# ocramz/rp-tree

Measured on AMD Instinct MI355X. Metric: forest-build vectors/s (1000000 x 128 dense f64, 32 trees; projection mode mfma = RPT_PROJ_MFMA, the API default RPT_PROJ_AUTO on f64 data is the exact-order kernel timed in `other_projection_mode`); kNN queries/s and recall@10 in `knn` / `recall_at_10`, higher is better.
Workload: dtype f64; 1 GPU; C2: 1000000 x 128 f64 two-Gaussian mixture, 32-tree forest, minLeaf 128, maxDepth 13, pnz 0.4746, k=10, 10000 queries; trees sharded 32/GPU, X replicated; projection_mode=mfma

## Files before the change

### rp-tree_amd/csrc/api.hip

```cpp
#include <cctype>
#include <cmath>
#include <cstdlib>
#include <cstring>
#include <limits>
#include <map>
#include <mutex>
#include <new>

#include "common.h"

namespace rpt {

static thread_local std::string g_err;
void set_error(const std::string& msg) { g_err = msg; }
int32_t fail(int32_t code, const std::string& msg) {
  g_err = msg;
  return code;
}

namespace {
struct Block {
  void* p;
  size_t bytes;
};
// ... 108 lines not shown

int32_t upload_async(rpt_ctx* ctx, void* dst_dev, const void* src_host, size_t bytes) {
  if (bytes == 0) return RPT_OK;
  void* stage = pin_alloc(ctx, bytes);
  if (!stage) {
    RPT_HIP(hipMemcpyAsync(dst_dev, src_host, bytes, hipMemcpyHostToDevice, ctx->stream));
    RPT_HIP(stream_sync(ctx->stream));
    return RPT_OK;
  }
  std::memcpy(stage, src_host, bytes);
  RPT_HIP(hipMemcpyAsync(dst_dev, stage, bytes, hipMemcpyHostToDevice, ctx->stream));
  return RPT_OK;
}

hipError_t ctx_sync(rpt_ctx* ctx) {
  const hipError_t e = stream_sync(ctx->stream);
  ctx->pin_off = 0;
  return e;
}

void dev_trim() {
  int dev = 0;
  (void)hipGetDevice(&dev);
  (void)hipDeviceSynchronize();
  std::lock_guard<std::mutex> lk(g_pool_mu);
  for (size_t i = 0; i < g_pool_pending.size();) {
    if (g_pool_pending[i].dev == dev) {
      (void)hipFree(g_pool_pending[i].p);
      g_pool_pending[i] = g_pool_pending.back();
      g_pool_pending.pop_back();
    } else {
      ++i;
    }
  }
  auto it = g_pool_free.find(dev);
  if (it != g_pool_free.end()) {
    for (Block& b : it->second) (void)hipFree(b.p);
    it->second.clear();
  }
}

void enumerate_topology(int64_t N, int32_t L, int32_t min_leaf, std::vector<Node>& out) {
  struct Item { int32_t level; int64_t heap, off, n; };
  std::vector<Item> stack;
  stack.push_back({0, 0, 0, N});
  while (!stack.empty()) {
    Item it = stack.back();
    stack.pop_back();
    bool leaf = is_leaf(it.level, it.n, L, min_leaf);
    out.push_back({it.level, it.heap, it.off, it.n, leaf});
    if (!leaf) {
      int64_t nh = it.n / 2;
      stack.push_back({it.level + 1, 2 * it.heap + 2, it.off + nh, it.n - nh});
      stack.push_back({it.level + 1, 2 * it.heap + 1, it.off, nh});
    }
  }
}

}

using namespace rpt;

static void prof_resolve(rpt_ctx* ctx);

namespace {
struct OptDesc {
  const char* name;
  int64_t rpt_options::*field;
};
const OptDesc kOptions[] = {
    {"no_stream", &rpt_options::no_stream},
    {"stream_maxnodes", &rpt_options::stream_maxnodes},
    {"stream_minper", &rpt_options::stream_minper},
    {"no_wmid", &rpt_options::no_wmid},
    {"no_midselect", &rpt_options::no_midselect},
    {"stream_big_node", &rpt_options::stream_big_node},
    {"no_wsub", &rpt_options::no_wsub},
    {"no_wsort", &rpt_options::no_wsort},
    {"no_wpack", &rpt_options::no_wpack},
    {"no_csub", &rpt_options::no_csub},
    {"no_codes", &rpt_options::no_codes},
    {"no_pcodes", &rpt_options::no_pcodes},
    {"proj_narrow", &rpt_options::proj_narrow},
    {"proj_bf16_f32", &rpt_options::proj_bf16_f32},
    {"proj_bf16_terms", &rpt_options::proj_bf16_terms},
    {"proj_bf16_codes", &rpt_options::proj_bf16_codes},
    {"proj_csr_nodense", &rpt_options::proj_csr_nodense},
    {"knn_wave", &rpt_options::knn_wave},
    {"knn_kp", &rpt_options::knn_kp},
    {"knn_no_pre32", &rpt_options::knn_no_pre32},
    {"knn_no_pre16", &rpt_options::knn_no_pre16},
    {"knn_kp16", &rpt_options::knn_kp16},
    {"knn_no_pre8", &rpt_options::knn_no_pre8},
    {"knn_kp8", &rpt_options::knn_kp8},
    {"knn_metric_exact", &rpt_options::knn_metric_exact},
    {"knn_csr_pre32", &rpt_options::knn_csr_pre32},
    {"knn_general", &rpt_options::knn_general},
    {"graph_general", &rpt_options::graph_general},
    {"graph_refine_general", &rpt_options::graph_refine_general},
    {"graph_search_nofilter", &rpt_options::graph_search_nofilter},
    {"knn_shard_old", &rpt_options::knn_shard_old},
    {"brute_csr_tile", &rpt_options::brute_csr_tile},
    {"comm_force_exchange", &rpt_options::comm_force_exchange},
    {"comm_inject_failure", &rpt_options::comm_inject_failure},
    {"comm_timeout_ms", &rpt_options::comm_timeout_ms},
    {"comm_stall_test", &rpt_options::comm_stall_test},
    {"tune0", &rpt_options::tune0},
    {"tune1", &rpt_options::tune1},
    {"tune2", &rpt_options::tune2},
    {"tune3", &rpt_options::tune3},
    {"debug_host", &rpt_options::debug_host},
    {"debug_stamps", &rpt_options::debug_stamps},
};
const OptDesc* find_option(const char* name) {
  if (!name) return nullptr;
  for (const OptDesc& o : kOptions)
    if (std::strcmp(o.name, name) == 0) return &o;
  return nullptr;
}
void options_from_env(rpt_options& opt) {
  for (const OptDesc& o : kOptions) {
    std::string env = "RPT_";
    for (const char* c = o.name; *c; ++c) env += (char)std::toupper((unsigned char)*c);
    if (const char* v = getenv(env.c_str())) {
      char* end = nullptr;
      const long long x = std::strtoll(v, &end, 10);
      opt.*(o.field) = (end && end != v) ? (int64_t)x : 1;
    }
  }
}

template <class F>
int32_t guarded(F&& body) noexcept {
  try {
    return body();
  } catch (const std::bad_alloc&) {
    try {
      return fail(RPT_E_NOMEM, "out of host memory");
    } catch (...) {
      return RPT_E_NOMEM;
    }
  } catch (const std::exception& e) {
    try {
      return fail(RPT_E_INTERNAL, std::string("internal error: ") + e.what());
    } catch (...) {
      return RPT_E_INTERNAL;
    }
  } catch (...) {
    return RPT_E_INTERNAL;
  }
}
}

extern "C" {

int32_t rpt_abi_version(void) { return RPT_ABI_VERSION; }
const char* rpt_last_error(void) { return g_err.c_str(); }

int32_t rpt_device_count(int32_t* count) {
  return guarded([&]() -> int32_t {
    RPT_ARG(count, "count is NULL");
    int c = 0;
    hipError_t e = hipGetDeviceCount(&c);
    if (e != hipSuccess) {
      *count = 0;
      return fail(RPT_E_HIP, std::string("hipGetDeviceCount: ") + hipGetErrorString(e));
// ... 1322 lines not shown
```

### rp-tree_amd/csrc/common.h

```cpp
#pragma once

#include <hip/hip_runtime.h>
#include <stdint.h>

#include <atomic>
#include <mutex>
#include <string>
#include <vector>

#include "../../include/rptree_hip.h"

namespace rpt {

void set_error(const std::string& msg);
int32_t fail(int32_t code, const std::string& msg);

#define RPT_HIP(expr)                                                                     \
  do {                                                                                    \
    hipError_t e__ = (expr);                                                              \
    if (e__ != hipSuccess)                                                                \
      return ::rpt::fail(RPT_E_HIP, std::string(#expr) + ": " + hipGetErrorString(e__));  \
  } while (0)

#define RPT_TRY(expr)             \
// ... 18 lines not shown
  return level >= L || n <= (int64_t)min_leaf;
}
void enumerate_topology(int64_t N, int32_t L, int32_t min_leaf, std::vector<Node>& out);

struct Seg {
  int64_t off;
  int32_t n;
  int32_t heap;
};

inline size_t dtype_size(int32_t dt) { return dt == RPT_F64 ? 8 : dt == RPT_F32 ? 4 : 2; }
inline int32_t proj_dtype(int32_t dt) { return dt == RPT_F64 ? RPT_F64 : RPT_F32; }

hipError_t dev_alloc(void** p, size_t bytes);
void dev_free(void* p);
void dev_trim();
void dev_set_stream(hipStream_t s);
hipError_t stream_sync(hipStream_t s);

struct DeviceOnce {
  std::mutex mu;
  std::atomic<unsigned long long> done{0};
  template <class F>
  int32_t run(int dev, F&& f) {
    const unsigned long long bit = 1ULL << (dev & 63);
    if (done.load(std::memory_order_acquire) & bit) return 0;
    std::lock_guard<std::mutex> lk(mu);
    if (done.load(std::memory_order_relaxed) & bit) return 0;
    const int32_t s = f();
    if (s == 0) done.fetch_or(bit, std::memory_order_release);
    return s;
  }
};

template <class T>
struct DevBuf {
  T* p = nullptr;
  size_t count = 0;
  ~DevBuf() { release(); }
  DevBuf() = default;
  DevBuf(const DevBuf&) = delete;
  DevBuf& operator=(const DevBuf&) = delete;
  void release() {
    if (p) dev_free(p);
    p = nullptr;
    count = 0;
  }
  int32_t alloc(size_t n) {
    release();
    if (n == 0) n = 1;
    hipError_t e = dev_alloc((void**)&p, n * sizeof(T));
    if (e != hipSuccess)
      return fail(RPT_E_NOMEM, std::string("hipMalloc failed: ") + hipGetErrorString(e));
    count = n;
    return RPT_OK;
  }
  int32_t ensure(size_t n) { return (n <= count && p) ? RPT_OK : alloc(n); }
};

}

enum { RPT_PROF_PROJECT = 0, RPT_PROF_SPLIT = 1, RPT_PROF_KNN_PLAN = 2, RPT_PROF_KNN_TOPK = 3,
       RPT_PROF_PROJECT_WIDE = 4, RPT_PROF_CLASSES = 5 };

struct rpt_prof_span {
  hipEvent_t a, b;
  int which;
};

struct rpt_options {
  int64_t no_stream = 0;
  int64_t stream_maxnodes = 0;
  int64_t stream_minper = 32768;
  int64_t no_wmid = 0;
  int64_t no_midselect = 0;
  int64_t stream_big_node = (int64_t)1 << 21;
  int64_t no_wsub = 0;
  int64_t no_wsort = 0;
  int64_t no_wpack = 0;
  int64_t no_csub = 0;
  int64_t no_codes = 0;
  int64_t no_pcodes = 0;
  int64_t proj_narrow = 0;
  int64_t proj_bf16_f32 = 0;
  int64_t proj_bf16_codes = 0;
  int64_t proj_bf16_terms = 0;
  int64_t proj_csr_nodense = 0;
  int64_t knn_wave = -1;
  int64_t knn_kp = 0;
  int64_t knn_no_pre32 = 0;
  int64_t knn_no_pre16 = 0;
  int64_t knn_kp16 = 0;
  int64_t knn_no_pre8 = 0;
  int64_t knn_kp8 = 0;
  int64_t knn_metric_exact = 0;
  int64_t knn_csr_pre32 = 0;
  int64_t knn_general = 0;
  int64_t graph_general = 0;
  int64_t graph_refine_general = 0;
  int64_t graph_search_nofilter = 0;
  int64_t brute_csr_tile = 0;
  int64_t knn_shard_old = 0;
  int64_t comm_force_exchange = 0;
  int64_t comm_inject_failure = 0;
  int64_t comm_timeout_ms = 0;
  int64_t comm_stall_test = 0;
  int64_t tune0 = 0, tune1 = 0, tune2 = 0, tune3 = 0;
  int64_t debug_host = 0;
  int64_t debug_stamps = 0;
};

struct rpt_ctx {
  rpt_options opt;
  int32_t device = 0;
  hipStream_t stream = nullptr;
  char* pin = nullptr;
  size_t pin_cap = 0, pin_off = 0;
  int64_t last_uncertified = 0;
  unsigned long long* metric_unc_dev = nullptr;
  bool metric_unc_pending = false;
  int64_t last_candidates = 0;
  int64_t last_retries = 0;
  int64_t last_graph_pairs = 0;
  void* refine_state_dev = nullptr;
  void* search_state_dev = nullptr;
  void* prepare_state_dev = nullptr;
  int32_t last_tier = 0;
  int64_t last_csub_redo = 0, last_csub_bad = 0;
  int32_t n_cu = 256;
  bool prof = false;
  std::vector<rpt_prof_span> spans;
  std::vector<hipEvent_t> prof_events;
  double prof_ms[RPT_PROF_CLASSES] = {0, 0, 0, 0, 0};
  int64_t prof_n[RPT_PROF_CLASSES] = {0, 0, 0, 0, 0};
};

namespace rpt {
struct ProfScope {
  rpt_ctx* ctx;
  rpt_prof_span sp;
  bool on;
  ProfScope(rpt_ctx* c, int which) : ctx(c), on(c->prof) {
    if (!on) return;
    sp.which = which;
    auto take = [&](hipEvent_t& e) {
      if (!ctx->prof_events.empty()) {
        e = ctx->prof_events.back();
        ctx->prof_events.pop_back();
        return true;
      }
      return hipEventCreate(&e) == hipSuccess;
    };
    if (!take(sp.a)) {
      on = false;
      return;
    }
    if (!take(sp.b)) {
      ctx->prof_events.push_back(sp.a);
      on = false;
      return;
    }
    (void)hipEventRecord(sp.a, ctx->stream);
  }
  ~ProfScope() {
    if (!on) return;
    (void)hipEventRecord(sp.b, ctx->stream);
// ... 120 lines not shown
```

### rp-tree_amd/csrc/project.hip

```cpp
#include <hip/hip_bf16.h>

#include <cstdlib>
#include <vector>

#include "common.h"
#include "codes.h"

namespace rpt {
namespace {

typedef double double4_t __attribute__((ext_vector_type(4)));
typedef float float4_t __attribute__((ext_vector_type(4)));

constexpr int kWave = 64;

template <class T>
struct Vec16;
template <>
struct Vec16<double> { typedef double type __attribute__((ext_vector_type(2))); };
template <>
struct Vec16<float> { typedef float type __attribute__((ext_vector_type(4))); };

template <class T>
__global__ void transpose_R(const double* __restrict__ R, int C, int d, int CB,
                            T* __restrict__ Rt) {
  int64_t total = (int64_t)((C + CB - 1) / CB) * d * CB;
  for (int64_t i = blockIdx.x * (int64_t)blockDim.x + threadIdx.x; i < total;
       i += (int64_t)gridDim.x * blockDim.x) {
    int c = (int)(i % CB);
    int k = (int)((i / CB) % d);
    int blk = (int)(i / ((int64_t)CB * d));
    int col = blk * CB + c;
    Rt[i] = col < C ? (T)R[(int64_t)col * d + k] : (T)0;
  }
}

__device__ inline double mul_rn(double a, double b) { return __dmul_rn(a, b); }
__device__ inline double add_rn(double a, double b) { return __dadd_rn(a, b); }
__device__ inline float mul_rn(float a, float b) { return __fmul_rn(a, b); }
__device__ inline float add_rn(float a, float b) { return __fadd_rn(a, b); }
__device__ inline double fma_rn(double a, double b, double c) { return __builtin_fma(a, b, c); }
__device__ inline float fma_rn(float a, float b, float c) { return __builtin_fmaf(a, b, c); }

template <class T, int CB, int KC>
__global__ __launch_bounds__(256) void proj_exact(const T* __restrict__ X, int64_t n, int d,
                                                  const T* __restrict__ Rt ,
                                                  T* __restrict__ P, int64_t ldp, int ncol) {
  constexpr int LDW = KC + 1;
  __shared__ T tile[4][kWave * LDW];
  const int lane = threadIdx.x & 63;
  const int wave = threadIdx.x >> 6;
  const int64_t row0 = ((int64_t)blockIdx.x * 4 + wave) * kWave;
  T* my = tile[wave];

  T acc[CB];
#pragma unroll
  for (int c = 0; c < CB; ++c) acc[c] = (T)0;

  const int nchunk = (d + KC - 1) / KC;
  for (int ch = nchunk - 1; ch >= 0; --ch) {
    const int k0 = ch * KC;
    const int klen = min(KC, d - k0);
    __syncthreads();
    for (int e = lane; e < kWave * KC; e += kWave) {
      int r = e / KC, k = e % KC;
      int64_t row = row0 + r;
      T v = (T)0;
      if (k < klen && row < n) v = X[row * d + k0 + k];
      my[r * LDW + k] = v;
    }
    __syncthreads();
    const T* rrow = Rt + (int64_t)k0 * CB;
    for (int k = klen - 1; k >= 0; --k) {
      const T x = my[lane * LDW + k];
      const T* rk = rrow + (int64_t)k * CB;
#pragma unroll
      for (int c = 0; c < CB; ++c) acc[c] = add_rn(mul_rn(rk[c], x), acc[c]);
    }
  }
  const int64_t row = row0 + lane;
  if (row < n) {
#pragma unroll
    for (int c = 0; c < CB; ++c)
      if (c < ncol) P[(int64_t)c * ldp + row] = acc[c];
  }
// ... 213 lines not shown
  const int hi = __builtin_amdgcn_mov_dpp((int)(b >> 32), 0xb1, 0xf, 0xf, true);
  return __longlong_as_double(((long long)hi << 32) | (unsigned int)lo);
}
__device__ __forceinline__ float lane_swap1(float x) {
  return __int_as_float(__builtin_amdgcn_mov_dpp(__float_as_int(x), 0xb1, 0xf, 0xf, true));
}

template <class TC, int CBT, bool CODES>
__device__ __forceinline__ void tile_store(const typename Mfma<TC>::acc_t (&acc)[CBT], TC* __restrict__ P,
                                           int64_t ldp, int c0, int ncol, int64_t row0, int64_t n,
                                           int lane, const CodeCtl<TC>* ctl, unsigned int cmask) {
  const int64_t r4 = row0 + 4 * (lane >> 4);
  if constexpr (sizeof(TC) == 8) {
    const bool whole = row0 + 15 < n && (ldp & 1) == 0 && ncol == CBT * 16;
    if (whole) {
      typedef double d2 __attribute__((ext_vector_type(2), aligned(16)));
      const int odd = lane & 1;
#pragma unroll
      for (int h = 0; h < CBT; ++h) {
        const double g0 = odd ? acc[h][0] : acc[h][2], g1 = odd ? acc[h][1] : acc[h][3];
        const double x0 = lane_swap1(g0), x1 = lane_swap1(g1);
        const int col = h * 16 + (lane & 15);
        TC* pe = P + (int64_t)(c0 + (col & ~1)) * ldp + r4 + 2 * odd;
        TC* po = pe + ldp;
        d2 ve, vo;
        if (odd) {
          ve = d2{x0, x1};
          vo = d2{acc[h][2], acc[h][3]};
        } else {
          ve = d2{acc[h][0], acc[h][1]};
          vo = d2{x0, x1};
        }
        *reinterpret_cast<d2*>(pe) = ve;
        *reinterpret_cast<d2*>(po) = vo;
      }
    }
    if (whole) goto codes;
  }
  if (r4 >= n) return;
  {
  const bool vec = r4 + 3 < n && (ldp & 3) == 0;
#pragma unroll
  for (int h = 0; h < CBT; ++h) {
    const int col = h * 16 + (lane & 15);
    if (col < ncol) {
      TC* p = P + (int64_t)(c0 + col) * ldp + r4;
      if (vec) {
        typename Vec4<TC>::type v;
#pragma unroll
        for (int r = 0; r < 4; ++r) v[r] = acc[h][r];
        *reinterpret_cast<typename Vec4<TC>::type*>(p) = v;
      } else {
#pragma unroll
        for (int r = 0; r < 4; ++r)
          if (r4 + r < n) p[r] = acc[h][r];
      }
    }
  }
  }
codes:
  if constexpr (CODES) {
    if (cmask == 0) return;
    const CodeCtl<TC> cc = *ctl;
    const CodeGeo<TC> g{cc.s, cc.b};
    const bool cvec = r4 + 3 < n && (cc.ld & 3) == 0;
#pragma unroll
    for (int h = 0; h < CBT; ++h)
      if ((cmask >> h) & 1u) {
        uint16_t* q = cc.base + (int64_t)(h * 16 + (lane & 15)) * cc.ld + r4;
        if (cvec) {
          code4_t v;
#pragma unroll
          for (int r = 0; r < 4; ++r) v[r] = code_of(acc[h][r], g);
          *reinterpret_cast<code4_t*>(q) = v;
        } else {
#pragma unroll
          for (int r = 0; r < 4; ++r)
            if (r4 + r < n) q[r] = code_of(acc[h][r], g);
        }
      }
  }
}

template <class TIn, class TC, int CBT, int KCH, int WAVES>
__global__ __launch_bounds__(WAVES * 64) void proj_mfma(const TIn* __restrict__ X, int64_t n,
                                                        int d, const double* __restrict__ R,
                                                        int c0, int ncol, TC* __restrict__ P,
                                                        int64_t ldp, int64_t ntiles) {
  constexpr int STEPS = KCH / 4;
  constexpr int LDW = KCH + 16 / (int)sizeof(TC);
  __shared__ __attribute__((aligned(16))) TC tile[WAVES][16 * LDW];
  const int lane = threadIdx.x & 63;
  const int wave = threadIdx.x >> 6;
  const int m = lane & 15, q = lane >> 4;
  TC* my = tile[wave];
  typedef typename Mfma<TC>::acc_t acc_t;

  const int nchunk = (d + KCH - 1) / KCH;
  TC a[CBT][STEPS];
  auto load_a = [&](int k0) {
#pragma unroll
    for (int h = 0; h < CBT; ++h) {
      const int col = h * 16 + m;
#pragma unroll
      for (int s = 0; s < STEPS; ++s) {
        const int k = k0 + 4 * s + q;
        a[h][s] = (col < ncol && k < d) ? (TC)R[(int64_t)(c0 + col) * d + k] : (TC)0;
      }
    }
  };
  if (nchunk == 1) load_a(0);

  const int64_t wave_global = (int64_t)blockIdx.x * WAVES + wave;
  const int64_t wave_stride = (int64_t)gridDim.x * WAVES;
  for (int64_t t = wave_global; t < ntiles; t += wave_stride) {
    const int64_t row0 = t * 16;
    acc_t acc[CBT];
#pragma unroll
    for (int h = 0; h < CBT; ++h) acc[h] = acc_t{0, 0, 0, 0};

    for (int ch = 0; ch < nchunk; ++ch) {
      const int k0 = ch * KCH;
      if (nchunk > 1) load_a(k0);
      constexpr int VEC = 16 / (int)sizeof(TIn);
      const bool vec_ok = (d % VEC) == 0;
      __builtin_amdgcn_wave_barrier();
      if (vec_ok) {
        for (int e = lane; e < 16 * (KCH / VEC); e += 64) {
          const int r = e / (KCH / VEC), kv = (e % (KCH / VEC)) * VEC;
          const int64_t row = row0 + r;
          TC v[VEC];
          if (row < n && k0 + kv < d) {
            struct alignas(16) Raw { TIn v[VEC]; };
            const Raw g = *reinterpret_cast<const Raw*>(X + row * d + k0 + kv);
#pragma unroll
            for (int j = 0; j < VEC; ++j) {
              if constexpr (sizeof(TIn) == sizeof(TC)) v[j] = (TC)g.v[j];
              else v[j] = (TC)to_f32<TIn>(g.v[j]);
            }
          } else {
#pragma unroll
            for (int j = 0; j < VEC; ++j) v[j] = (TC)0;
          }
#pragma unroll
          for (int j = 0; j < VEC; ++j) my[r * LDW + kv + j] = v[j];
        }
      } else {
        for (int e = lane; e < 16 * KCH; e += 64) {
          const int r = e / KCH, k = e % KCH;
          const int64_t row = row0 + r;
          TC v = (TC)0;
          if (row < n && k0 + k < d) {
            if constexpr (sizeof(TIn) == sizeof(TC)) v = (TC)X[row * d + k0 + k];
            else v = (TC)to_f32<TIn>(X[row * d + k0 + k]);
          }
          my[r * LDW + k] = v;
        }
      }
      __builtin_amdgcn_wave_barrier();
      __builtin_amdgcn_fence(__ATOMIC_ACQ_REL, "wavefront");
#pragma unroll
      for (int s = 0; s < STEPS; ++s) {
        const TC b = my[m * LDW + 4 * s + q];
#pragma unroll
        for (int h = 0; h < CBT; ++h) acc[h] = Mfma<TC>::run(a[h][s], b, acc[h]);
      }
    }
    const int64_t row = row0 + m;
    if (row < n) {
#pragma unroll
      for (int h = 0; h < CBT; ++h)
#pragma unroll
        for (int r = 0; r < 4; ++r) {
          const int col = h * 16 + Mfma<TC>::row_of(lane, r);
          if (col < ncol) P[(int64_t)(c0 + col) * ldp + row] = acc[h][r];
        }
    }
  }
}

template <class TC>
__global__ void pad_A_kernel(const double* __restrict__ R, int C, int d, int D, int nblk, int cbt,
                             int col0, int k0, TC* __restrict__ Apad ) {
  const int steps = D / 4;
  const int64_t total = (int64_t)nblk * cbt * steps * 64;
  for (int64_t i = blockIdx.x * (int64_t)blockDim.x + threadIdx.x; i < total;
       i += (int64_t)gridDim.x * blockDim.x) {
    const int lane = (int)(i & 63);
    const int s = (int)((i >> 6) % steps);
    const int h = (int)((i / (64 * (int64_t)steps)) % cbt);
    const int blk = (int)(i / (64 * (int64_t)steps * cbt));
    const int col = col0 + blk * 16 * cbt + h * 16 + (lane & 15);
    const int k = k0 + 4 * s + (lane >> 4);
    Apad[i] = (col < C && k < d) ? (TC)R[(int64_t)col * d + k] : (TC)0;
  }
}

template <class TIn, class TC, int D, int CBT, bool CODES = false>
__device__ __forceinline__ void proj_fast_body(const TIn* __restrict__ X, int64_t n,
                                               const TC* __restrict__ Apad, int c0,
                                               int ncol, TC* __restrict__ P,
                                               int64_t ldp, int64_t ntiles,
                                               int64_t ldx ,
                                               int accumulate ,
                                               int kvalid ,
                                               uint16_t* __restrict__ Cd ,
                                               int64_t ldc,
                                               const unsigned long long* __restrict__ cmm,
                                               int cL, int cLc ) {
  constexpr int STEPS = D / 4;
  constexpr int PIECE = 16 / (int)sizeof(TIn);
  constexpr int PIECES_PER_ROW = D / PIECE;
  __shared__ CodeCtl<TC> cctl;
  unsigned int cmask = 0;
  if constexpr (CODES) {
    if (threadIdx.x == 0) {
      const CodeGeo<TC> g = code_geo<TC>(cmm[0], cmm[1]);
      cctl = CodeCtl<TC>{Cd + (int64_t)c0 * ldc, ldc, g.s, g.b};
    }
    cmask = code_lane_mask<CBT>(threadIdx.x & 63, c0, ncol, cL, cLc);
    __syncthreads();
  }
  constexpr int NP = 16 * PIECES_PER_ROW / 64;
  constexpr int LDW = D + 16 / (int)sizeof(TC);
  static_assert((16 * PIECES_PER_ROW) % 64 == 0, "tile must be a multiple of 64 pieces");
  __shared__ __attribute__((aligned(16))) TC tile[4][16 * LDW];
  const int lane = threadIdx.x & 63;
  const int wave = threadIdx.x >> 6;
  const int m = lane & 15, q = lane >> 4;
  TC* my = tile[wave];
  typedef typename Mfma<TC>::acc_t acc_t;
  struct alignas(16) Raw { TIn v[PIECE]; };

  TC a[CBT][STEPS];
#pragma unroll
  for (int h = 0; h < CBT; ++h)
#pragma unroll
    for (int s = 0; s < STEPS; ++s) a[h][s] = Apad[(h * STEPS + s) * 64 + lane];

  const int64_t wave_global = (int64_t)blockIdx.x * 4 + wave;
  const int64_t wave_stride = (int64_t)gridDim.x * 4;
  const int64_t last_row = n - 1;

  Raw stage[NP];
  auto issue = [&](int64_t t) {
    const int64_t row0 = t * 16;
#pragma unroll
    for (int i = 0; i < NP; ++i) {
      const int p = i * 64 + lane;
      int64_t row = row0 + p / PIECES_PER_ROW;
      row = row < last_row ? row : last_row;
      if ((p % PIECES_PER_ROW) * PIECE < kvalid)
        stage[i] = *reinterpret_cast<const Raw*>(X + row * ldx + (p % PIECES_PER_ROW) * PIECE);
      else
        stage[i] = Raw{};
    }
  };
  auto commit = [&]() {
#pragma unroll
    for (int i = 0; i < NP; ++i) {
      const int p = i * 64 + lane;
      TC* dst = my + (p / PIECES_PER_ROW) * LDW + (p % PIECES_PER_ROW) * PIECE;
#pragma unroll
      for (int j = 0; j < PIECE; ++j) {
        if constexpr (sizeof(TIn) == sizeof(TC)) dst[j] = (TC)stage[i].v[j];
        else dst[j] = (TC)to_f32<TIn>(stage[i].v[j]);
      }
    }
  };

  int64_t t = wave_global;
  if (t < ntiles) issue(t);
  while (t < ntiles) {
    commit();
    const int64_t tn = t + wave_stride;
    if (tn < ntiles) issue(tn);
    acc_t acc[CBT];
#pragma unroll
    for (int h = 0; h < CBT; ++h) acc[h] = acc_t{0, 0, 0, 0};
    if (accumulate) tile_load<TC, CBT>(acc, P, ldp, c0, ncol, t * 16, n, lane);
    const int mp = Mfma<TC>::point_of_m(m);
#pragma unroll
    for (int s = 0; s < STEPS; ++s) {
      const TC b = my[mp * LDW + 4 * s + q];
#pragma unroll
      for (int h = 0; h < CBT; ++h) acc[h] = Mfma<TC>::run(b, a[h][s], acc[h]);
    }
    tile_store<TC, CBT, CODES>(acc, P, ldp, c0, ncol, t * 16, n, lane, &cctl, cmask);
    t = tn;
  }
}

template <class TIn, class TC, int D, int CBT, bool CODES = false>
__global__ __launch_bounds__(256, 2) void proj_mfma_fast(const TIn* __restrict__ X, int64_t n,
                                                         const TC* __restrict__ Apad, int c0, int ncol,
                                                         TC* __restrict__ P, int64_t ldp, int64_t ntiles,
                                                         int64_t ldx, int accumulate, int kvalid,
                                                         uint16_t* __restrict__ Cd, int64_t ldc,
                                                         const unsigned long long* __restrict__ cmm,
                                                         int cL, int cLc) {
  proj_fast_body<TIn, TC, D, CBT, CODES>(X, n, Apad, c0, ncol, P, ldp, ntiles, ldx, accumulate, kvalid, Cd,
                                         ldc, cmm, cL, cLc);
}

template <class TIn, class TC, int D>
__global__ __launch_bounds__(256, 2) void proj_mfma_fast_groups(const TIn* __restrict__ X, int64_t n,
                                                                const TC* __restrict__ Apad, int C,
                                                                TC* __restrict__ P, int64_t ldp,
                                                                int64_t ntiles, int64_t ldx, int kvalid) {
  const int c0 = (int)blockIdx.y * 32;
  const int ncol = C - c0 < 32 ? C - c0 : 32;
  proj_fast_body<TIn, TC, D, 2, false>(X, n, Apad + (size_t)blockIdx.y * 2 * (D / 4) * 64, c0, ncol, P, ldp,
                                       ntiles, ldx, 0, kvalid, nullptr, 0, nullptr, 1, 0);
}

template <class TC, int D, int CBT, int KS, int WPB>
constexpr size_t wide_smem_bytes() {
  return ((size_t)CBT * (D / 4) * 64 + (size_t)WPB * 16 * (D / KS + 16 / sizeof(TC))) * sizeof(TC) +
         sizeof(CodeCtl<TC>);
}

template <class TIn, class TC, int D, int CBT, int KS, int WPB, bool CODES = false>
__global__ __launch_bounds__(WPB * 64, 1) void proj_mfma_wide(const TIn* __restrict__ X, int64_t n,
                                                         const TC* __restrict__ Apad, int c0,
                                                         int ncol, TC* __restrict__ P,
                                                         int64_t ldp, int64_t ntiles,
                                                         int64_t ldx ,
                                                         int accumulate ,
                                                         int kvalid ,
                                                         uint16_t* __restrict__ Cd ,
                                                         int64_t ldc,
                                                         const unsigned long long* __restrict__ cmm,
                                                         int cL, int cLc ) {
  constexpr int STEPS = D / 4, SSTEPS = STEPS / KS, KW = D / KS;
  constexpr int PIECE = 16 / (int)sizeof(TIn);
  constexpr int PPR = KW / PIECE;
  constexpr int NP = 16 * PPR / 64;
  constexpr int LDW = KW + 16 / (int)sizeof(TC);
  static_assert((16 * PPR) % 64 == 0 && NP >= 1, "slice must be a multiple of 64 pieces");
  static_assert(KS % 2 == 0, "two register stages alternate per slice");
  extern __shared__ __attribute__((aligned(16))) unsigned char wide_smem[];
  TC* As = reinterpret_cast<TC*>(wide_smem);
  TC* tiles = As + (size_t)CBT * STEPS * 64;
  CodeCtl<TC>* cctl = reinterpret_cast<CodeCtl<TC>*>(tiles + (size_t)WPB * 16 * LDW);
  const int lane = threadIdx.x & 63;
  const int wave = threadIdx.x >> 6;
  const int m = lane & 15, q = lane >> 4;
  TC* my = tiles + (size_t)wave * 16 * LDW;
  typedef typename Mfma<TC>::acc_t acc_t;
  struct alignas(16) Raw { TIn v[PIECE]; };

  for (int i = threadIdx.x; i < CBT * STEPS * 64; i += WPB * 64) As[i] = Apad[i];
  unsigned int cmask = 0;
  if constexpr (CODES) {
    if (threadIdx.x == 0) {
      const CodeGeo<TC> g = code_geo<TC>(cmm[0], cmm[1]);
      *cctl = CodeCtl<TC>{Cd + (int64_t)c0 * ldc, ldc, g.s, g.b};
    }
    cmask = code_lane_mask<CBT>(lane, c0, ncol, cL, cLc);
  }
  __syncthreads();

  const int64_t wave_global = (int64_t)blockIdx.x * WPB + wave;
  const int64_t wave_stride = (int64_t)gridDim.x * WPB;
  const int64_t last_row = n - 1;

  Raw stg0[NP], stg1[NP];
  auto issue = [&](Raw (&stage)[NP], int64_t t, int slice) {
    const int64_t row0 = t * 16;
#pragma unroll
    for (int i = 0; i < NP; ++i) {
      const int p = i * 64 + lane;
      int64_t row = row0 + p / PPR;
      row = row < last_row ? row : last_row;
      if (slice * KW + (p % PPR) * PIECE < kvalid)
        stage[i] = *reinterpret_cast<const Raw*>(X + row * ldx + slice * KW + (p % PPR) * PIECE);
      else
        stage[i] = Raw{};
    }
  };
  auto commit = [&](const Raw (&stage)[NP]) {
#pragma unroll
    for (int i = 0; i < NP; ++i) {
      const int p = i * 64 + lane;
      TC* dst = my + (p / PPR) * LDW + (p % PPR) * PIECE;
#pragma unroll
      for (int j = 0; j < PIECE; ++j) {
        if constexpr (sizeof(TIn) == sizeof(TC)) dst[j] = (TC)stage[i].v[j];
        else dst[j] = (TC)to_f32<TIn>(stage[i].v[j]);
      }
    }
  };

  int64_t t = wave_global;
  if (t < ntiles) {
    issue(stg0, t, 0);
    issue(stg1, t, 1);
  }
  while (t < ntiles) {
    const int64_t tn = t + wave_stride;
    acc_t acc[CBT];
#pragma unroll
    for (int h = 0; h < CBT; ++h) acc[h] = acc_t{0, 0, 0, 0};
    if (accumulate) tile_load<TC, CBT>(acc, P, ldp, c0, ncol, t * 16, n, lane);
    const int mp = Mfma<TC>::point_of_m(m);
#pragma unroll
    for (int sl = 0; sl < KS; ++sl) {
      if (sl % 2 == 0) commit(stg0);
      else commit(stg1);
      if (sl + 2 < KS) {
        if (sl % 2 == 0) issue(stg0, t, sl + 2);
        else issue(stg1, t, sl + 2);
      } else if (tn < ntiles) {
        if (sl % 2 == 0) issue(stg0, tn, sl + 2 - KS);
        else issue(stg1, tn, sl + 2 - KS);
      }
      if (sl * KW < kvalid) {
#pragma unroll
        for (int s = 0; s < SSTEPS; ++s) {
          const TC b = my[mp * LDW + 4 * s + q];
#pragma unroll
          for (int h = 0; h < CBT; ++h)
            acc[h] = Mfma<TC>::run(b, As[(h * STEPS + sl * SSTEPS + s) * 64 + lane], acc[h]);
        }
      }
    }
    tile_store<TC, CBT, CODES>(acc, P, ldp, c0, ncol, t * 16, n, lane, cctl, cmask);
    t = tn;
  }
}

typedef __bf16 bf16x8 __attribute__((ext_vector_type(8)));
typedef float f32x4 __attribute__((ext_vector_type(4)));
constexpr int kB3KC = 2;

__global__ void split_A_bf16x3(const double* __restrict__ R, int d, int c0, int ncol, int cbt,
                               int nch, int kc , int np ,
                               uint4* __restrict__ out) {
  const int per_chunk = kc * np * cbt * 64;
  const int total = nch * kc * cbt * 64;
  for (int i = blockIdx.x * blockDim.x + threadIdx.x; i < total; i += gridDim.x * blockDim.x) {
    const int lane = i & 63;
    int r = i >> 6;
    const int mt = r % cbt;
    r /= cbt;
    const int ks = r % kc, ch = r / kc;
    const int col = mt * 16 + (lane & 15);
    const int k0 = (ch * kc + ks) * 32 + 8 * (lane >> 4);
    unsigned int w[3][4] = {{0, 0, 0, 0}, {0, 0, 0, 0}, {0, 0, 0, 0}};
    for (int j = 0; j < 8; ++j) {
      double v = (col < ncol && k0 + j < d) ? R[(int64_t)(c0 + col) * d + k0 + j] : 0.0;
      for (int p3 = 0; p3 < 3; ++p3) {
        const __hip_bfloat16 b = __float2bfloat16((float)v);
        v -= (double)__bfloat162float(b);
        const unsigned int bits = (unsigned int)__builtin_bit_cast(unsigned short, b);
        w[p3][j >> 1] |= bits << ((j & 1) * 16);
      }
    }
    for (int p3 = 0; p3 < np; ++p3)
      out[(size_t)ch * per_chunk + ((ks * np + p3) * cbt + mt) * 64 + lane] =
          make_uint4(w[p3][0], w[p3][1], w[p3][2], w[p3][3]);
  }
}

template <int CBT, int NT , bool RESIDENT ,
          int WAVES , class TP = float ,
          int NTERM = 1 ,
          int NP = 3 , int KC = kB3KC ,
          bool CODES = false ,
          int RD = 4 >
__global__ __launch_bounds__(WAVES * 64) void proj_bf16x3(
    const __hip_bfloat16* __restrict__ X, int64_t n, int d, const uint4* __restrict__ Aimg,
    int nch , int c0, int ncol, TP* __restrict__ P, int64_t ldp, int64_t ntiles,
    uint16_t* __restrict__ Cd, int64_t ldc, const unsigned long long* __restrict__ cmm, int cL, int cLc) {
  extern __shared__ __attribute__((aligned(16))) uint4 lds_a[];
  constexpr int CH16 = KC * NP * CBT * 64;
  constexpr int kB3NT = NT, kB3Pts = WAVES * NT * 16, NTHR = WAVES * 64;
  constexpr int ST = CH16 / NTHR;
  static_assert(KC == 2 || KC == 4, "the B ring is addressed by (chunk parity, k-step)");
  static_assert(NT % 2 == 0 && CH16 % NTHR == 0, "point tiles are stored in pairs; whole staging rounds");
// ... 373 lines not shown
        v.v[e] = ok ? val[idx] : (T)0;
      }
    }
  };
  auto column = [&](int j, int e) { return 4 * NP * ((rho + j) & (NR - 1)) + NP * q + e; };
  auto sums = [&](int64_t gg, T (&dst)[NR][NP]) {
    const int64_t r = gg * 16 + (lane >> 2);
#pragma unroll
    for (int j = 0; j < NR; ++j)
#pragma unroll
      for (int e = 0; e < NP; ++e) {
        const int c = column(j, e);
        dst[j][e] = (gg < ngroups && r < n && c < ncol) ? P[(int64_t)c * ldp + r] : (T)0;
      }
  };

  int64_t a, b, an, bn;
  range(g, a, b);
  int64_t j0 = b;
  C4 cc;
  V4 vc;
  fetch(a, j0, cc, vc);
  range(g + wave_stride, an, bn);
  T acc[NR][NP], nat[NR][NP];
#pragma unroll
  for (int j = 0; j < NR; ++j)
#pragma unroll
    for (int e = 0; e < NP; ++e) acc[j][e] = nat[j][e] = (T)0;
  if (part == 2) sums(g, acc);
  for (;;) {
    const bool more = __any(j0 - 16 > a);
    const int64_t gn = g + wave_stride;
    const bool last = !more && gn >= ngroups;
    const int64_t na = more ? a : an, nj0 = more ? j0 - 16 : bn;
    C4 cn;
    V4 vn;
    if (!last) fetch(na, nj0, cn, vn);
    if (!more && !last && part == 2) sums(gn, nat);
    int mycolb[4];
    T myval[4];
#pragma unroll
    for (int e = 0; e < 4; ++e) {
      mycolb[e] = (cc.v[e] - k_lo) * G::kRowBytes;
      myval[e] = vc.v[e];
    }
    const int64_t rem = j0 - a;
    if (__any(rem >= 1)) {
      csr_group32<T, 3, FUSED>(mycolb, myval, rp, acc);
      if (__any(rem >= 5)) {
        csr_group32<T, 2, FUSED>(mycolb, myval, rp, acc);
        if (__any(rem >= 9)) {
          csr_group32<T, 1, FUSED>(mycolb, myval, rp, acc);
          if (__any(rem >= 13)) csr_group32<T, 0, FUSED>(mycolb, myval, rp, acc);
        }
      }
    }
    if (!more) {
      const int64_t row = g * 16 + (lane >> 2);
      if (row < n) {
#pragma unroll
        for (int j = 0; j < NR; ++j)
#pragma unroll
          for (int e = 0; e < NP; ++e) {
            const int c = column(j, e);
            if (c < ncol) P[(int64_t)c * ldp + row] = acc[j][e];
          }
      }
      if (last) break;
      g = gn;
      a = an;
      b = bn;
      range(g + wave_stride, an, bn);
#pragma unroll
      for (int j = 0; j < NR; ++j)
#pragma unroll
        for (int e = 0; e < NP; ++e) acc[j][e] = nat[j][e];
    }
    j0 = nj0;
    cc = cn;
    vc = vn;
  }
}

template <class TIn, class TC, int D, int CBT, int KS>
int32_t launch_wide(rpt_ctx* ctx, const rpt_dataset* ds, int k0, int kvalid, int accumulate, int c0,
                    int ncol, const TC* Ab, TC* P, int64_t ntiles, int64_t blocks,
                    const CodeOut* co ) {
  constexpr int WPB = 8;
  constexpr size_t smem = wide_smem_bytes<TC, D, CBT, KS, WPB>();
  static DeviceOnce attr_once;
  RPT_TRY(attr_once.run(ctx->device, [&]() -> int32_t {
    RPT_HIP(hipFuncSetAttribute(
        reinterpret_cast<const void*>(&proj_mfma_wide<TIn, TC, D, CBT, KS, WPB, false>),
        hipFuncAttributeMaxDynamicSharedMemorySize, (int)smem));
    RPT_HIP(hipFuncSetAttribute(
        reinterpret_cast<const void*>(&proj_mfma_wide<TIn, TC, D, CBT, KS, WPB, true>),
        hipFuncAttributeMaxDynamicSharedMemorySize, (int)smem));
    return RPT_OK;
  }));
  if (co)
    hipLaunchKernelGGL((proj_mfma_wide<TIn, TC, D, CBT, KS, WPB, true>), dim3((unsigned)blocks),
                       dim3(WPB * 64), smem, ctx->stream, (const TIn*)ds->X + k0, ds->n, Ab, c0,
                       ncol, P, ds->n, ntiles, (int64_t)ds->d, accumulate, kvalid, co->codes, co->ld,
                       co->mm, co->L, co->Lc);
  else
    hipLaunchKernelGGL((proj_mfma_wide<TIn, TC, D, CBT, KS, WPB, false>), dim3((unsigned)blocks),
                       dim3(WPB * 64), smem, ctx->stream, (const TIn*)ds->X + k0, ds->n, Ab, c0,
                       ncol, P, ds->n, ntiles, (int64_t)ds->d, accumulate, kvalid,
                       (uint16_t*)nullptr, (int64_t)0, (const unsigned long long*)nullptr, 1, 0);
  return RPT_OK;
}

template <class TIn, class TC>
int32_t launch_mfma(rpt_ctx* ctx, const rpt_dataset* ds, const double* R_dev, int32_t C,
                    TC* P, const CodeOut* co, bool* codes_written) {
  const int64_t n = ds->n;
  const int64_t ntiles = (n + 15) / 16;
  constexpr int kPiece = 16 / (int)sizeof(TIn);
  if (ds->d % kPiece == 0) {
    constexpr int D = 128;
    const int nkc = (ds->d + D - 1) / D;
    if (nkc == 1 && C > 32 && !co && n <= 65536 && !ctx->opt.proj_narrow) {
      const int ngrp = (C + 31) / 32;
      const size_t frag1 = (size_t)(D / 4) * 64;
      DevBuf<TC> Ag;
      RPT_TRY(Ag.alloc((size_t)ngrp * 2 * frag1));
      hipLaunchKernelGGL(pad_A_kernel<TC>, dim3(64), dim3(256), 0, ctx->stream, R_dev, C, ds->d, D, ngrp, 2,
                         0, 0, Ag.p);
      int64_t bx = (ntiles + 3) / 4;
      const int64_t capx = ((int64_t)ctx->n_cu * 8 + ngrp - 1) / ngrp;
      if (bx > capx) bx = capx;
      if (bx < 1) bx = 1;
      ProfScope pn(ctx, RPT_PROF_PROJECT);
      hipLaunchKernelGGL((proj_mfma_fast_groups<TIn, TC, D>), dim3((unsigned)bx, (unsigned)ngrp), dim3(256), 0,
                         ctx->stream, (const TIn*)ds->X, n, Ag.p, C, P, n, ntiles, (int64_t)ds->d, ds->d);
      RPT_HIP(hipGetLastError());
      return RPT_OK;
    }
    struct Pass {
      int c0, ncol, tiles;
    };
    std::vector<Pass> passes;
    constexpr int KS8 = sizeof(TC) == 8 ? 8 : 4;
    {
      const bool wide_ok = !ctx->opt.proj_narrow;
      int c0 = 0;
      while (c0 < C) {
        const int left = C - c0;
        int take, tiles;
        if (!wide_ok || left <= 32) {
          take = left < 32 ? left : 32;
          tiles = 0;
        } else if (left <= 64) {
          take = left;
          tiles = 4;
        } else if (left <= 96) {
          take = left;
          tiles = 6;
        } else if (left <= 128) {
          take = left;
          tiles = 8;
        } else if (sizeof(TC) == 4 && left <= 160) {
          take = left;
          tiles = left <= 144 ? 9 : 10;
        } else {
          take = 96;
          tiles = 6;
        }
        passes.push_back(Pass{c0, take, tiles});
        c0 += take;
      }
    }
    const size_t frag = (size_t)(D / 4) * 64;
    size_t total_tiles = 0;
    for (const Pass& ps : passes) total_tiles += ps.tiles ? ps.tiles : 2;
    DevBuf<TC> Afrag;
    RPT_TRY(Afrag.alloc(total_tiles * nkc * frag));
    {
      size_t off = 0;
      for (int kc = 0; kc < nkc; ++kc)
        for (const Pass& ps : passes) {
          const int tl = ps.tiles ? ps.tiles : 2;
          hipLaunchKernelGGL(pad_A_kernel<TC>, dim3(16), dim3(256), 0, ctx->stream, R_dev, C, ds->d,
                             D, 1, tl, ps.c0, kc * D, Afrag.p + off);
          off += (size_t)tl * frag;
        }
    }
    int64_t wblocks = (ntiles + 7) / 8;
    if (wblocks > ctx->n_cu) wblocks = ctx->n_cu;
    int64_t blocks = (ntiles + 3) / 4;
    const int64_t cap = (int64_t)ctx->n_cu * 2;
    if (blocks > cap) blocks = cap;
    size_t off = 0;
    for (int kc = 0; kc < nkc; ++kc) {
      const int k0 = kc * D, accumulate = kc > 0;
      const int kvalid = ds->d - k0 < D ? ds->d - k0 : D;
      const CodeOut* cop = (co && kc == nkc - 1) ? co : nullptr;
      for (const Pass& ps : passes) {
        const TC* Ab = Afrag.p + off;
        off += (size_t)(ps.tiles ? ps.tiles : 2) * frag;
        if (ps.tiles) {
          ProfScope pw(ctx, RPT_PROF_PROJECT_WIDE);
          switch (ps.tiles) {
            case 10:
            case 9:
              if constexpr (sizeof(TC) == 4) {
                if (ps.tiles == 10)
                  RPT_TRY((launch_wide<TIn, TC, D, 10, 4>(ctx, ds, k0, kvalid, accumulate, ps.c0, ps.ncol, Ab, P,
                                                          ntiles, wblocks, cop)));
                else
                  RPT_TRY((launch_wide<TIn, TC, D, 9, 4>(ctx, ds, k0, kvalid, accumulate, ps.c0, ps.ncol, Ab, P,
                                                         ntiles, wblocks, cop)));
              }
              break;
            case 8:
              RPT_TRY((launch_wide<TIn, TC, D, 8, KS8>(ctx, ds, k0, kvalid, accumulate, ps.c0,
                                                       ps.ncol, Ab, P, ntiles, wblocks, cop)));
              break;
            case 6:
              RPT_TRY((launch_wide<TIn, TC, D, 6, 4>(ctx, ds, k0, kvalid, accumulate, ps.c0,
                                                     ps.ncol, Ab, P, ntiles, wblocks, cop)));
              break;
            default:
              RPT_TRY((launch_wide<TIn, TC, D, 4, 2>(ctx, ds, k0, kvalid, accumulate, ps.c0,
                                                     ps.ncol, Ab, P, ntiles, wblocks, cop)));
          }
        } else {
          ProfScope pn(ctx, RPT_PROF_PROJECT);
#define RPT_FAST(CBT_, CODES_)                                                                  \
  hipLaunchKernelGGL((proj_mfma_fast<TIn, TC, D, CBT_, CODES_>), dim3((unsigned)blocks), dim3(256), \
                     0, ctx->stream, (const TIn*)ds->X + k0, n, Ab, ps.c0, ps.ncol, P, n, ntiles,  \
                     (int64_t)ds->d, accumulate, kvalid, cop ? cop->codes : (uint16_t*)nullptr,    \
                     cop ? cop->ld : (int64_t)0, cop ? cop->mm : (const unsigned long long*)nullptr, \
                     cop ? cop->L : 1, cop ? cop->Lc : 0)
          if (ps.ncol > 16) {
            if (cop) RPT_FAST(2, true);
            else RPT_FAST(2, false);
          } else {
            if (cop) RPT_FAST(1, true);
            else RPT_FAST(1, false);
          }
#undef RPT_FAST
        }
      }
    }
    RPT_HIP(hipGetLastError());
    if (co && codes_written) *codes_written = true;
    return RPT_OK;
  }
  constexpr int WAVES = 4;
  int64_t blocks = (ntiles + WAVES - 1) / WAVES;
  const int64_t cap = (int64_t)ctx->n_cu * 8;
  if (blocks > cap) blocks = cap;
  if (blocks < 1) blocks = 1;
  for (int c0 = 0; c0 < C; c0 += 32) {
    const int ncol = C - c0 < 32 ? C - c0 : 32;
    ProfScope ps(ctx, RPT_PROF_PROJECT);
    if (ncol > 16)
      hipLaunchKernelGGL((proj_mfma<TIn, TC, 2, 128, WAVES>), dim3((unsigned)blocks),
                         dim3(WAVES * 64), 0, ctx->stream, (const TIn*)ds->X, n, ds->d, R_dev,
                         c0, ncol, P, n, ntiles);
    else
      hipLaunchKernelGGL((proj_mfma<TIn, TC, 1, 128, WAVES>), dim3((unsigned)blocks),
                         dim3(WAVES * 64), 0, ctx->stream, (const TIn*)ds->X, n, ds->d, R_dev,
                         c0, ncol, P, n, ntiles);
  }
  RPT_HIP(hipGetLastError());
  return RPT_OK;
}
// ... 368 lines not shown
```

Baseline: 223.5 million vectors/s.

## Add opt-in software-pipelined wide MFMA projection and batch A-fragment padding

Adds a PIPE variant of the wide MFMA projection kernel, enabled by a new `proj_wide_pipe` option. In that variant, each full 16-row tile's stores of projections and codes are interleaved into the next tile's MFMA K-loop, using paired-lane f64 vector stores and buffer-store codes, so global stores overlap compute. It also replaces the per-pass, per-K-chunk `pad_A_kernel` launches with a single 2D launch covering all passes and K chunks. This launch change relies on every non-final pass spanning a whole number of 16-column tiles and returns an internal error otherwise. The pipelined path is off by default, so with default settings only the launch batching is active.

```diff
diff --git a/rp-tree_amd/csrc/api.hip b/rp-tree_amd/csrc/api.hip
--- a/rp-tree_amd/csrc/api.hip
+++ b/rp-tree_amd/csrc/api.hip
@@ -214,6 +214,7 @@
     {"no_codes", &rpt_options::no_codes},
     {"no_pcodes", &rpt_options::no_pcodes},
     {"proj_narrow", &rpt_options::proj_narrow},
+    {"proj_wide_pipe", &rpt_options::proj_wide_pipe},
     {"proj_bf16_f32", &rpt_options::proj_bf16_f32},
     {"proj_bf16_terms", &rpt_options::proj_bf16_terms},
     {"proj_bf16_codes", &rpt_options::proj_bf16_codes},
diff --git a/rp-tree_amd/csrc/common.h b/rp-tree_amd/csrc/common.h
--- a/rp-tree_amd/csrc/common.h
+++ b/rp-tree_amd/csrc/common.h
@@ -124,6 +124,7 @@
   int64_t no_codes = 0;
   int64_t no_pcodes = 0;
   int64_t proj_narrow = 0;
+  int64_t proj_wide_pipe = 0;
   int64_t proj_bf16_f32 = 0;
   int64_t proj_bf16_codes = 0;
   int64_t proj_bf16_terms = 0;
diff --git a/rp-tree_amd/csrc/project.hip b/rp-tree_amd/csrc/project.hip
--- a/rp-tree_amd/csrc/project.hip
+++ b/rp-tree_amd/csrc/project.hip
@@ -1,6 +1,7 @@
 #include <hip/hip_bf16.h>
 
 #include <cstdlib>
+#include <type_traits>
 #include <vector>
 
 #include "common.h"
@@ -380,6 +381,41 @@
   }
 }
 
+typedef unsigned int code_words_t __attribute__((ext_vector_type(2)));
+template <class TC, bool CODES>
+__device__ __forceinline__ void tile_store_step(const typename Mfma<TC>::acc_t& a, TC* __restrict__ p,
+                                                int64_t ldp, int lane, __amdgpu_buffer_rsrc_t crs, int coff,
+                                                const CodeCtl<TC>* ctl) {
+  if constexpr (sizeof(TC) == 8) {
+    typedef double d2 __attribute__((ext_vector_type(2), aligned(16)));
+    const int odd = lane & 1;
+    const double g0 = odd ? a[0] : a[2], g1 = odd ? a[1] : a[3];
+    const double x0 = lane_swap1(g0), x1 = lane_swap1(g1);
+    d2 ve, vo;
+    if (odd) {
+      ve = d2{x0, x1};
+      vo = d2{a[2], a[3]};
+    } else {
+      ve = d2{a[0], a[1]};
+      vo = d2{x0, x1};
+    }
+    *reinterpret_cast<d2*>(p) = ve;
+    *reinterpret_cast<d2*>(p + ldp) = vo;
+  } else {
+    typename Vec4<TC>::type v;
+#pragma unroll
+    for (int r = 0; r < 4; ++r) v[r] = a[r];
+    *reinterpret_cast<typename Vec4<TC>::type*>(p) = v;
+  }
+  if constexpr (CODES) {
+    const CodeGeo<TC> g{ctl->s, ctl->b};
+    unsigned int c[4];
+#pragma unroll
+    for (int r = 0; r < 4; ++r) c[r] = code_of(a[r], g);
+    __builtin_amdgcn_raw_buffer_store_b64(code_words_t{c[0] | (c[1] << 16), c[2] | (c[3] << 16)}, crs, coff, 0, 0);
+  }
+}
+
 template <class TIn, class TC, int CBT, int KCH, int WAVES>
 __global__ __launch_bounds__(WAVES * 64) void proj_mfma(const TIn* __restrict__ X, int64_t n,
                                                         int d, const double* __restrict__ R,
@@ -482,6 +518,8 @@
                              int col0, int k0, TC* __restrict__ Apad ) {
   const int steps = D / 4;
   const int64_t total = (int64_t)nblk * cbt * steps * 64;
+  k0 += (int)blockIdx.y * D;
+  Apad += blockIdx.y * total;
   for (int64_t i = blockIdx.x * (int64_t)blockDim.x + threadIdx.x; i < total;
        i += (int64_t)gridDim.x * blockDim.x) {
     const int lane = (int)(i & 63);
@@ -618,7 +656,7 @@
          sizeof(CodeCtl<TC>);
 }
 
-template <class TIn, class TC, int D, int CBT, int KS, int WPB, bool CODES = false>
+template <class TIn, class TC, int D, int CBT, int KS, int WPB, bool CODES = false, bool PIPE = false>
 __global__ __launch_bounds__(WPB * 64, 1) void proj_mfma_wide(const TIn* __restrict__ X, int64_t n,
                                                          const TC* __restrict__ Apad, int c0,
                                                          int ncol, TC* __restrict__ P,
@@ -664,14 +702,14 @@
   const int64_t last_row = n - 1;
 
   Raw stg0[NP], stg1[NP];
-  auto issue = [&](Raw (&stage)[NP], int64_t t, int slice) {
+  auto issue = [&](Raw (&stage)[NP], int64_t t, int slice, bool whole_rows = false) {
     const int64_t row0 = t * 16;
 #pragma unroll
     for (int i = 0; i < NP; ++i) {
       const int p = i * 64 + lane;
       int64_t row = row0 + p / PPR;
       row = row < last_row ? row : last_row;
-      if (slice * KW + (p % PPR) * PIECE < kvalid)
+      if (whole_rows || slice * KW + (p % PPR) * PIECE < kvalid)
         stage[i] = *reinterpret_cast<const Raw*>(X + row * ldx + slice * KW + (p % PPR) * PIECE);
       else
         stage[i] = Raw{};
@@ -694,6 +732,80 @@
   if (t < ntiles) {
     issue(stg0, t, 0);
     issue(stg1, t, 1);
+  }
+  if constexpr (PIPE) {
+    const bool pipe_ok = !accumulate && kvalid == D && ncol == CBT * 16 &&
+                         ldp % (sizeof(TC) == 8 ? 2 : 4) == 0 &&
+                         (!CODES || ((ldc & 3) == 0 && ldc < ((int64_t)1 << 25)));
+    const int64_t nfull = n >> 4;
+    if (pipe_ok && t < nfull) {
+      int64_t tu = (int64_t)blockIdx.x * WPB + __builtin_amdgcn_readfirstlane(wave);
+      const int mp = Mfma<TC>::point_of_m(m);
+      TC* const pl = sizeof(TC) == 8 ? P + (int64_t)(c0 + (m & ~1)) * ldp + 4 * q + 2 * (lane & 1)
+                                     : P + (int64_t)(c0 + m) * ldp + 4 * q;
+      const int coff = (int)(((int64_t)m * ldc + 4 * q) * 2);
+      constexpr int kNoCode = (int)0x80000000u;
+      constexpr int SP = STEPS / CBT;
+      static_assert(SP >= 1, "one drain step per K step at most");
+      auto ktile = [&](acc_t (&acc)[CBT], const acc_t (&dr)[CBT], auto DR, int64_t tt, int64_t tp) {
+        const int64_t tn = tt + wave_stride;
+#pragma unroll
+        for (int h = 0; h < CBT; ++h) acc[h] = acc_t{0, 0, 0, 0};
+        TC* pd = pl + tp * 16;
+        uint16_t* cd = Cd + (int64_t)c0 * ldc + tp * 16;
+#pragma unroll
+        for (int sl = 0; sl < KS; ++sl) {
+          if (sl % 2 == 0) commit(stg0);
+          else commit(stg1);
+          if (sl + 2 < KS) {
+            if (sl % 2 == 0) issue(stg0, tt, sl + 2, true);
+            else issue(stg1, tt, sl + 2, true);
+          } else if (tn < ntiles) {
+            if (sl % 2 == 0) issue(stg0, tn, sl + 2 - KS, true);
+            else issue(stg1, tn, sl + 2 - KS, true);
+          }
+#pragma unroll
+          for (int s = 0; s < SSTEPS; ++s) {
+            const TC b = my[mp * LDW + 4 * s + q];
+#pragma unroll
+            for (int h = 0; h < CBT; ++h)
+              acc[h] = Mfma<TC>::run(b, As[(h * STEPS + sl * SSTEPS + s) * 64 + lane], acc[h]);
+            if constexpr (decltype(DR)::value) {
+              const int g = sl * SSTEPS + s + 1;
+              if (g % SP == 0 && g / SP <= CBT) {
+                const int h = g / SP - 1;
+                const __amdgpu_buffer_rsrc_t crs =
+                    __builtin_amdgcn_make_buffer_rsrc(cd + (int64_t)h * 16 * ldc, 0, 0x7fffffff, 0x00020000);
+                tile_store_step<TC, CODES>(dr[h], pd + (int64_t)h * 16 * ldp, ldp, lane, crs,
+                                           ((cmask >> h) & 1u) ? coff : kNoCode, cctl);
+              }
+              __builtin_amdgcn_sched_barrier(0x1 | 0x20 | 0x80);
+            }
+          }
+        }
+      };
+      acc_t acc0[CBT], acc1[CBT];
+      ktile(acc0, acc1, std::false_type{}, tu, tu);
+      int64_t tp = tu;
+      tu += wave_stride;
+      for (;;) {
+        if (tu >= nfull) {
+          tile_store<TC, CBT, CODES>(acc0, P, ldp, c0, ncol, tp * 16, n, lane, cctl, cmask);
+          break;
+        }
+        ktile(acc1, acc0, std::true_type{}, tu, tp);
+        tp = tu;
+        tu += wave_stride;
+        if (tu >= nfull) {
+          tile_store<TC, CBT, CODES>(acc1, P, ldp, c0, ncol, tp * 16, n, lane, cctl, cmask);
+          break;
+        }
+        ktile(acc0, acc1, std::true_type{}, tu, tp);
+        tp = tu;
+        tu += wave_stride;
+      }
+      t = tu;
+    }
   }
   while (t < ntiles) {
     const int64_t tn = t + wave_stride;
@@ -1233,33 +1345,46 @@
   }
 }
 
-template <class TIn, class TC, int D, int CBT, int KS>
-int32_t launch_wide(rpt_ctx* ctx, const rpt_dataset* ds, int k0, int kvalid, int accumulate, int c0,
-                    int ncol, const TC* Ab, TC* P, int64_t ntiles, int64_t blocks,
-                    const CodeOut* co ) {
+template <class TIn, class TC, int D, int CBT, int KS, bool PIPE>
+int32_t launch_wide_as(rpt_ctx* ctx, const rpt_dataset* ds, int k0, int kvalid, int accumulate, int c0,
+                       int ncol, const TC* Ab, TC* P, int64_t ntiles, int64_t blocks,
+                       const CodeOut* co ) {
   constexpr int WPB = 8;
   constexpr size_t smem = wide_smem_bytes<TC, D, CBT, KS, WPB>();
   static DeviceOnce attr_once;
   RPT_TRY(attr_once.run(ctx->device, [&]() -> int32_t {
     RPT_HIP(hipFuncSetAttribute(
-        reinterpret_cast<const void*>(&proj_mfma_wide<TIn, TC, D, CBT, KS, WPB, false>),
+        reinterpret_cast<const void*>(&proj_mfma_wide<TIn, TC, D, CBT, KS, WPB, false, PIPE>),
         hipFuncAttributeMaxDynamicSharedMemorySize, (int)smem));
     RPT_HIP(hipFuncSetAttribute(
-        reinterpret_cast<const void*>(&proj_mfma_wide<TIn, TC, D, CBT, KS, WPB, true>),
+        reinterpret_cast<const void*>(&proj_mfma_wide<TIn, TC, D, CBT, KS, WPB, true, PIPE>),
         hipFuncAttributeMaxDynamicSharedMemorySize, (int)smem));
     return RPT_OK;
   }));
   if (co)
-    hipLaunchKernelGGL((proj_mfma_wide<TIn, TC, D, CBT, KS, WPB, true>), dim3((unsigned)blocks),
+    hipLaunchKernelGGL((proj_mfma_wide<TIn, TC, D, CBT, KS, WPB, true, PIPE>), dim3((unsigned)blocks),
                        dim3(WPB * 64), smem, ctx->stream, (const TIn*)ds->X + k0, ds->n, Ab, c0,
                        ncol, P, ds->n, ntiles, (int64_t)ds->d, accumulate, kvalid, co->codes, co->ld,
                        co->mm, co->L, co->Lc);
   else
-    hipLaunchKernelGGL((proj_mfma_wide<TIn, TC, D, CBT, KS, WPB, false>), dim3((unsigned)blocks),
+    hipLaunchKernelGGL((proj_mfma_wide<TIn, TC, D, CBT, KS, WPB, false, PIPE>), dim3((unsigned)blocks),
                        dim3(WPB * 64), smem, ctx->stream, (const TIn*)ds->X + k0, ds->n, Ab, c0,
                        ncol, P, ds->n, ntiles, (int64_t)ds->d, accumulate, kvalid,
                        (uint16_t*)nullptr, (int64_t)0, (const unsigned long long*)nullptr, 1, 0);
   return RPT_OK;
+}
+
+template <class TC>
+constexpr bool kWidePipe = sizeof(TC) == 8;
+template <class TIn, class TC, int D, int CBT, int KS>
+int32_t launch_wide(rpt_ctx* ctx, const rpt_dataset* ds, int k0, int kvalid, int accumulate, int c0,
+                    int ncol, const TC* Ab, TC* P, int64_t ntiles, int64_t blocks, const CodeOut* co) {
+  const int64_t pipe = ctx->opt.proj_wide_pipe;
+  if (pipe >= 2 || (pipe == 1 && kWidePipe<TC>))
+    return launch_wide_as<TIn, TC, D, CBT, KS, true>(ctx, ds, k0, kvalid, accumulate, c0, ncol, Ab, P, ntiles,
+                                                     blocks, co);
+  return launch_wide_as<TIn, TC, D, CBT, KS, false>(ctx, ds, k0, kvalid, accumulate, c0, ncol, Ab, P, ntiles,
+                                                    blocks, co);
 }
 
 template <class TIn, class TC>
@@ -1327,15 +1452,14 @@
     for (const Pass& ps : passes) total_tiles += ps.tiles ? ps.tiles : 2;
     DevBuf<TC> Afrag;
     RPT_TRY(Afrag.alloc(total_tiles * nkc * frag));
+    for (size_t i = 0; i + 1 < passes.size(); ++i)
+      if (passes[i].ncol != 16 * (passes[i].tiles ? passes[i].tiles : 2)) return RPT_E_INTERNAL;
     {
-      size_t off = 0;
-      for (int kc = 0; kc < nkc; ++kc)
-        for (const Pass& ps : passes) {
-          const int tl = ps.tiles ? ps.tiles : 2;
-          hipLaunchKernelGGL(pad_A_kernel<TC>, dim3(16), dim3(256), 0, ctx->stream, R_dev, C, ds->d,
-                             D, 1, tl, ps.c0, kc * D, Afrag.p + off);
-          off += (size_t)tl * frag;
-        }
+      const size_t words = total_tiles * frag;
+      unsigned bx = (unsigned)((words + 255) / 256);
+      if (bx > 64) bx = 64;
+      hipLaunchKernelGGL(pad_A_kernel<TC>, dim3(bx, (unsigned)nkc), dim3(256), 0, ctx->stream, R_dev, C, ds->d,
+                         D, 1, (int)total_tiles, 0, 0, Afrag.p);
     }
     int64_t wblocks = (ntiles + 7) / 8;
     if (wblocks > ctx->n_cu) wblocks = ctx->n_cu;
```

Measured after the change: 223.1 million vectors/s. About the same (-0.2%).
